# heli-sudoo/HKD-MPC

Measured on AMD Instinct MI355X. Metric: batched DDP iters/sec (fwd+bwd), 4-phase 200-knot HKD fp64, batch=4096, higher is better.
Workload: dtype f64

## Files before the change

hkd-mpc_amd/csrc/hsddp_api.cpp:

```cpp
#include <hip/hip_runtime.h>

#include <algorithm>
#include <chrono>
#include <cctype>
#include <cmath>
#include <cstdio>
#include <cstdlib>
#include <cstring>
#include <fstream>
#include <map>
#include <sstream>
#include <string>
#include <vector>

#include "../../include/hsddp.h"
#include "hsddp_internal.h"
#include "hsddp_mpc.h"

using namespace hsddp;

static thread_local std::string g_err;

static int fail(int code, const std::string &msg)
{
// ... 122 lines not shown
    if (s == "true" || s == "1") v = 1;
    else if (s == "false" || s == "0") v = 0;
    else return fail(HSDDP_ERR_IO, "conversion of data failed (" + k + ")");
    return HSDDP_OK;
}

extern "C" int hsddp_load_settings(const char *path, hsddp_options *o)
{
    if (!path || !o) return fail(HSDDP_ERR_ARG, "null argument");
    std::map<std::string, std::string> m;
    int rc = parse_info(path, m);
    if (rc) return rc;
    hsddp_options t = *o;
#define N_(k) if ((rc = get_num(m, "ddp." #k, t.k))) return rc
#define I_(k) if ((rc = get_int(m, "ddp." #k, t.k))) return rc
#define B_(k) if ((rc = get_bool(m, "ddp." #k, t.k))) return rc
    N_(alpha); N_(gamma); N_(update_penalty); N_(update_relax); N_(update_ReB);
    I_(max_DDP_iter); I_(max_AL_iter); I_(max_DDP_iter_runtime); I_(max_AL_iter_runtime);
    N_(cost_thresh); N_(tconstr_thresh); N_(pconstr_thresh); N_(dynamics_feas_thresh);
    N_(merit_rho); N_(merit_scale); N_(merit_offset);
    B_(AL_active); B_(ReB_active); B_(MS); I_(nsteps_per_node);
#undef N_
#undef I_
#undef B_
    *o = t;
    return HSDDP_OK;
}

extern "C" int hsddp_load_constraint_params(const char *path, hsddp_constraint_params *cp)
{
    if (!path || !cp) return fail(HSDDP_ERR_ARG, "null argument");
    std::map<std::string, std::string> m;
    int rc = parse_info(path, m);
    if (rc) return rc;
    hsddp_constraint_params t = *cp;
    if ((rc = get_num(m, "GRF_ReB.delta", t.grf_delta)) || (rc = get_num(m, "GRF_ReB.delta_min", t.grf_delta_min)) ||
        (rc = get_num(m, "GRF_ReB.eps", t.grf_eps)) || (rc = get_num(m, "Swing_ReB.delta", t.swing_delta)) ||
        (rc = get_num(m, "Swing_ReB.delta_min", t.swing_delta_min)) || (rc = get_num(m, "Swing_ReB.eps", t.swing_eps)) ||
        (rc = get_num(m, "TD_AL.sigma", t.td_sigma)) || (rc = get_num(m, "TD_AL.lambda", t.td_lambda)) ||
        (rc = get_num(m, "TD_AL.sigma_max", t.td_sigma_max)))
        return rc;
    *cp = t;
    return HSDDP_OK;
}

struct hsddp_handle_t {
    bool slots_fresh = false;
    bool reb_at_init = true;
    hsddp_problem_desc desc;
    hsddp_options opt;
    Params p;
    Bufs d;
    hipStream_t stream = nullptr;
    int *host_counter = nullptr;
    std::vector<hipEvent_t> events;
    struct IterGraph {
        hipGraphExec_t exec = nullptr;
        Params p;
        Bufs d;
        double alpha = 0;
        int par = 0;
    } iter_graph[8];
    int iter_graph_next = 0;
    std::vector<std::vector<int>> shift_keep;
    bool shift_overflow_pending = false;
    size_t scratch_reserved = 0;
    hipEvent_t iter_done[2] = {nullptr, nullptr};
    std::vector<void *> allocs;
    size_t bytes = 0;
    int Bref = 1;
    bool have_problem = false;
    std::vector<int> contacts;
    bool contacts_current = false;
    void *scratch = nullptr;
    size_t scratch_bytes = 0;
    std::vector<int> reach_end;
    size_t S_cap = 0;
    void *spare_K = nullptr;
    double *spare_reb_delta = nullptr, *spare_reb_eps = nullptr, *spare_al_sigma = nullptr, *spare_al_lambda = nullptr;
    int *spare_td_mask = nullptr;
    double *spare_cf_u = nullptr;
    int *spare_cf_flag = nullptr;
    double *shift_stage = nullptr;
    bool need_inputs = false;
    double *ref_table = nullptr;
    int ref_n = 0;
    float ref_dt = 0;
    bool refs_on_device = false;
    bool ref_cols_stale = true;
    std::vector<hsddp_quad_state> table_host;
    std::vector<int> win_start;
    int win_len = 0;
    float dt_sim = 0, t_cur = 0;
    std::vector<double> durations;
    int retry_cap_alloc = 0, retry_m_alloc = 0;
    float *hist = nullptr;
    std::vector<Layout> lays;
    std::vector<int> reach_el;
    double *value0 = nullptr;
    hsddp_mpc_command *cmd_dev[2] = {nullptr, nullptr}, *cmd_host[2] = {nullptr, nullptr};
    hipStream_t copy_stream = nullptr;
    hipEvent_t cmd_ready[2] = {nullptr, nullptr}, cmd_copied[2] = {nullptr, nullptr};
    char *cmd_in_host[2] = {nullptr, nullptr};
    size_t cmd_in_bytes[2] = {0, 0};
    int cmd_next = 0;
};

static int scratch(hsddp_handle h, size_t bytes, char **out)
{
    if (bytes > h->scratch_bytes) {
        if (h->scratch) hipFree(h->scratch);
        h->scratch = nullptr;
        h->scratch_bytes = 0;
        hipError_t e = hipMalloc(&h->scratch, bytes);
// ... 137 lines not shown
        p.N[i] = desc->horizons[i]; p.s0[i] = s; p.k0[i] = k;
        s += p.N[i] + 1; k += p.N[i];
    }
    p.S = s; p.Kc = k;
    p.ref_per_element = desc->ref_per_element ? 1 : 0;
    p.fp32 = desc->riccati_fp32 ? 1 : 0;
    h->Bref = p.ref_per_element ? p.B : 1;
    fill_params(h);
    for (int i = 0; i < p.P; ++i) p.ss[i] = p.N[i] + 1;
    p.has_tail = 0;
    h->reach_end.assign(p.P, 0);
    h->S_cap = (size_t)p.Kc + HSDDP_MAX_PHASES;
    const size_t B = p.B, S = h->S_cap, Kc = p.Kc, P = HSDDP_MAX_PHASES, Br = h->Bref;
    Bufs &d = h->d;
    int *contacts; double *x0, *rx, *ru, *rf;
    int rc = 0;
    if ((rc = dalloc(h, contacts, B * (P + 1) * 4)) || (rc = dalloc(h, x0, B * NX)) || (rc = dalloc(h, rx, Br * S * NX)) ||
        (rc = dalloc(h, ru, Br * S * NX)) || (rc = dalloc(h, rf, Br * S * 12)) || (rc = dalloc(h, d.ref_t, REF_COLS * Br * S)) ||
        (rc = dalloc(h, d.X3, 3 * B * S * NX)) ||
        (rc = dalloc(h, d.D3, 3 * B * S * NX)) || (rc = dalloc(h, d.U3, 3 * B * Kc * NX)) || (rc = dalloc(h, d.sel, B)) ||
        (rc = dalloc(h, d.cf_u, B * Kc * 12)) || (rc = dalloc(h, d.cf_flag, B * Kc)) ||
        (rc = dalloc(h, d.dX, B * S * NX)) ||
        (rc = dalloc(h, d.dU, B * Kc * NX)) ||
        (rc = dalloc(h, d.du, B * Kc * NX)) || (rc = dalloc(h, d.dbg, B * 16)) ||
        (p.fp32 ? ((rc = dalloc(h, d.K32, B * Kc * KCW)) || (rc = dalloc(h, d.lq32, B * Kc * LQW32)) ||
                   (rc = dalloc(h, d.def32, B * S * NX)))
                : ((rc = dalloc(h, d.K, B * Kc * KCW)) || (rc = dalloc(h, d.lq, B * Kc * LQW)))) ||
        (rc = dalloc(h, d.term, B * P * TW)) || (rc = dalloc(h, d.reb_delta, B * Kc * 20)) ||
        (rc = dalloc(h, d.reb_eps, B * Kc * 20)) || (rc = dalloc(h, d.al_sigma, B * P * MTD * 4)) ||
        (rc = dalloc(h, d.al_lambda, B * P * MTD * 4)) || (rc = dalloc(h, d.td_mask, B * P * MTD)) ||
        (rc = dalloc(h, d.term_h, B * P * 4)) ||
        (rc = dalloc(h, d.slot_cost, B * S)) || (rc = dalloc(h, d.slot_feas, B * S)) || (rc = dalloc(h, d.slot_viol, B * S)) ||
        (rc = dalloc(h, d.slot_div, B * S)) || (rc = dalloc(h, d.el, B)) || (rc = dalloc(h, d.counter, 8)) || (rc = dalloc(h, d.ls_live, LS_LIVE)) ||
        (rc = dalloc(h, (Layout *&)d.lay, B)) || (rc = dalloc(h, (int *&)d.pairs, 2 * B + 2))) {
        hsddp_destroy(h);
        return rc;
    }
    d.contacts = contacts; d.x0 = x0; d.ref_x = rx; d.ref_u = ru; d.ref_foot = rf;
    d.ref_tw = Br * S;
    d.xs3 = B * S * NX;
    d.us3 = B * Kc * NX;
    d.rows3 = (int)(B * S);
    d.urows3 = (int)(B * Kc);
    {
        const char *seq = std::getenv("HSDDP_SEQUENTIAL_RETRY");
        const char *capenv = std::getenv("HSDDP_RETRY_CAP");
        const size_t per_elem = (size_t)std::max(1, p.retry_m) * Kc * (KCW * (p.fp32 ? 4 : 8) + NX * 8 + 4);
        size_t cap = std::min<size_t>(std::min<size_t>(128, B), std::max<size_t>(2, ((size_t)256 << 20) / per_elem));
        if (capenv && std::atoi(capenv) > 0) cap = std::min<size_t>(cap, (size_t)std::atoi(capenv));
        const size_t M = (seq && seq[0] == '1') ? 0 : p.retry_m, n = cap * M;
        if (M > 0) {
            void *rk;
            if ((rc = dalloc(h, d.retry_list, cap)) || (rc = dalloc(h, d.retry_count, 1)) ||
                (rc = dalloc(h, d.retry_flag, n)) || (rc = dalloc(h, d.retry_dU, n * Kc * NX)) ||
                (rc = dalloc(h, d.retry_dv, n)) ||
                (rc = p.fp32 ? dalloc(h, (float *&)rk, n * Kc * KCW) : dalloc(h, (double *&)rk, n * Kc * KCW))) {
                hsddp_destroy(h);
                return rc;
            }
            d.retry_K = rk;
            h->retry_cap_alloc = (int)cap;
            h->retry_m_alloc = (int)M;
            fill_params(h);
        }
    }
    if (hipStreamCreateWithFlags(&h->stream, hipStreamNonBlocking) != hipSuccess ||
        hipHostMalloc((void **)&h->host_counter, 16 * sizeof(int), 0) != hipSuccess) {
        hsddp_destroy(h);
        return fail(HSDDP_ERR_DEVICE, "stream / pinned allocation failed");
    }
    if ((rc = ensure_history(h))) {
        hsddp_destroy(h);
        return rc;
    }
    launch_init_params(p, d, h->stream);
    launch_reset_elements(p, d, h->stream);
    if (hipStreamSynchronize(h->stream) != hipSuccess) {
        hsddp_destroy(h);
        return fail(HSDDP_ERR_DEVICE, "kernel launch failed at create (is the library built for this GPU?)");
    }
    *out = h;
    return HSDDP_OK;
}

extern "C" int hsddp_destroy(hsddp_handle h)
{
    if (!h) return HSDDP_OK;
    hipSetDevice(h->desc.device);
    if (h->stream) hipStreamSynchronize(h->stream);
    for (void *p : h->allocs) hipFree(p);
    if (h->scratch) hipFree(h->scratch);
    if (h->ref_table) hipFree(h->ref_table);
    if (h->hist) hipFree(h->hist);
    if (h->value0) hipFree(h->value0);

    for (auto &g : h->iter_graph)
        if (g.exec) hipGraphExecDestroy(g.exec);
    for (hipEvent_t e : h->iter_done)
        if (e) hipEventDestroy(e);
    if (h->host_counter) hipHostFree(h->host_counter);
    if (h->copy_stream) hipStreamSynchronize(h->copy_stream);
    for (int q = 0; q < 2; ++q) {
        if (h->cmd_dev[q]) hipFree(h->cmd_dev[q]);
        if (h->cmd_host[q]) hipHostFree(h->cmd_host[q]);
        if (h->cmd_ready[q]) hipEventDestroy(h->cmd_ready[q]);
        if (h->cmd_copied[q]) hipEventDestroy(h->cmd_copied[q]);
        if (h->cmd_in_host[q]) hipHostFree(h->cmd_in_host[q]);
    }
    if (h->copy_stream) hipStreamDestroy(h->copy_stream);
    for (hipEvent_t e : h->events) hipEventDestroy(e);
    if (h->stream) hipStreamDestroy(h->stream);
    delete h;
    return HSDDP_OK;
}

extern "C" int hsddp_validate_options(const hsddp_options *o)
{
    if (!o) return fail(HSDDP_ERR_ARG, "null argument");
    if (!(o->alpha > 0 && o->alpha < 1)) return fail(HSDDP_ERR_ARG, "alpha must lie in (0, 1)");
    if (o->max_AL_iter < 0 || o->max_DDP_iter < 0) return fail(HSDDP_ERR_ARG, "negative iteration budget");
    if (!(o->update_regularization > 1))
        return fail(HSDDP_ERR_ARG, "update_regularization must exceed 1 (the regularisation schedule would never end)");
    int m = 0;
    for (double mu = 0;; ++m) {
        mu = std::fmax(mu * o->update_regularization, 1e-03);
        if (mu > 1e2) break;
        if (m >= HSDDP_MAX_REG_ATTEMPTS)
            return fail(HSDDP_ERR_ARG, "update_regularization too close to 1: more than HSDDP_MAX_REG_ATTEMPTS "
                                       "regularisation retries per failed sweep");
    }
    return HSDDP_OK;
}

extern "C" int hsddp_set_options(hsddp_handle h, const hsddp_options *o)
{
    if (!h || !o) return fail(HSDDP_ERR_ARG, "null argument");
    int rc = hsddp_validate_options(o);
    if (rc) return rc;
    if (1 + (long)std::max(0, o->max_AL_iter) * std::max(0, o->max_DDP_iter) > (1L << 20))
        return fail(HSDDP_ERR_ARG, "max_AL_iter * max_DDP_iter exceeds the solver-info history (2^20 entries)");
    const hsddp_options old = h->opt;
    h->opt = *o;
    if ((rc = ensure_history(h))) {
        h->opt = old;
        return rc;
    }
    fill_params(h);
    return HSDDP_OK;
}

static int set_layouts(hsddp_handle h, const std::vector<Layout> &lays)
{
    h->slots_fresh = false;
    Params &p = h->p;
    const int B = p.B;
    int Pmax = 0, Smax = 0, tail = 0;
    for (auto &L : lays) { Pmax = std::max(Pmax, L.P); Smax = std::max(Smax, L.S); tail |= L.has_tail; }
    std::map<std::vector<int>, std::vector<int>> groups;
    for (int b = 0; b < B; ++b) {
        std::vector<int> key(lays[b].N, lays[b].N + lays[b].P);
        key.push_back(-1);
        key.insert(key.end(), lays[b].ss, lays[b].ss + lays[b].P);
        groups[key].push_back(b);
// ... 365 lines not shown
static int count_active(hsddp_handle h, int which, int &n)
{
    HIPCHK(hipMemsetAsync(h->d.counter, 0, 4 * sizeof(int), h->stream));
    launch_count(h->p, h->d, which, h->stream);
    HIPCHK(hipMemcpyAsync(h->host_counter, h->d.counter, 4 * sizeof(int), hipMemcpyDeviceToHost, h->stream));
    HIPCHK(hipStreamSynchronize(h->stream));
    n = h->host_counter[which];
    return HSDDP_OK;
}

static int solve_check(hsddp_handle h)
{
    if (!h) return fail(HSDDP_ERR_ARG, "null handle");
    if (!h->have_problem) return fail(HSDDP_ERR_ARG, "upload the problem first");
    if (h->need_inputs) return fail(HSDDP_ERR_ARG, "the layout changed (hsddp_shift): call hsddp_update_problem first");
    HIPCHK(hipSetDevice(h->desc.device));
    return HSDDP_OK;
}

static std::vector<double> ls_steps(double alpha)
{
    std::vector<double> trials;
    for (double eps = 1; eps > 1e-3; eps *= alpha) trials.push_back(eps);
    return trials;
}

static void sync_ref_columns(hsddp_handle h)
{
    if (!h->ref_cols_stale) return;
    launch_ref_columns(h->p, h->d, h->Bref, h->stream);
    h->ref_cols_stale = false;
}

static void begin_launches(hsddp_handle h)
{
    if (h->p.trace) hipMemsetAsync(h->d.dbg, 0, (size_t)h->p.B * 16 * sizeof(unsigned long long), h->stream);
    sync_ref_columns(h);
    launch_reset_elements(h->p, h->d, h->stream);
    launch_rollout(h->p, h->d, 0.0, 0, 1, -1, h->stream);
    launch_decide(h->p, h->d, 0.0, 0, 1, -1, h->stream);
    h->slots_fresh = true;
}

static void iteration_launches(hsddp_handle h, const std::vector<double> &trials, Timer &tm)
{
    const Params &p = h->p;
    const Bufs &d = h->d;
    hipStream_t st = h->stream;
    hipEvent_t e0;
    tm.begin(0, e0);
    {
        Params pl = p;
        pl.lq_slots = h->slots_fresh ? 0 : 1;
        launch_lq(pl, d, st);
    }
    tm.end(0, e0);
    tm.begin(1, e0);
    launch_riccati(p, d, st);
    tm.end(1, e0);
    if (!p.ms0) {
        tm.begin(4, e0);
        launch_lin_rollout(p, d, st);
        tm.end(4, e0);
    }
    tm.begin(2, e0);
    for (size_t t = 0; t < trials.size(); ++t) {
        launch_rollout(p, d, trials[t], t + 1 == trials.size(), 0, (int)t, st);
        launch_decide(p, d, trials[t], t + 1 == trials.size(), 0, (int)t, st);
    }
    tm.end(2, e0);
    h->slots_fresh = true;
}

static bool graphs_enabled()
{
    const char *e = std::getenv("HSDDP_NO_GRAPH");
    return !(e && *e && *e != '0');
}

static int graph_launch(hsddp_handle h, const std::vector<double> &trials, int par)
{
    Params pl = h->p;
    pl.lq_slots = h->slots_fresh ? 0 : 1;
    hsddp_handle_t::IterGraph *hit = nullptr;
    for (auto &c : h->iter_graph)
        if (c.exec && c.par == par && !std::memcmp(&c.p, &pl, sizeof(Params)) &&
            !std::memcmp(&c.d, &h->d, sizeof(Bufs)) && c.alpha == h->opt.alpha)
            hit = &c;
    if (!hit) {
        auto &g = h->iter_graph[h->iter_graph_next];
        h->iter_graph_next = (h->iter_graph_next + 1) % 8;
        if (g.exec) {
            HIPCHK(hipStreamSynchronize(h->stream));
            HIPCHK(hipGraphExecDestroy(g.exec));
        }
        g.exec = nullptr;
        HIPCHK(hipStreamBeginCapture(h->stream, hipStreamCaptureModeThreadLocal));
        Timer off{h->stream, false, &h->events};
        iteration_launches(h, trials, off);
        launch_count(h->p, h->d, 1, h->stream);
        hipError_t e = hipMemcpyAsync(h->host_counter + 8 + 4 * par, h->d.counter, 4 * sizeof(int), hipMemcpyDeviceToHost,
                               h->stream);
        hipGraph_t graph = nullptr;
        const hipError_t ec = hipStreamEndCapture(h->stream, &graph);
        if (e == hipSuccess) e = ec;
        if (e == hipSuccess) e = hipGraphInstantiate(&g.exec, graph, nullptr, nullptr, 0);
        if (graph) hipGraphDestroy(graph);
        if (e != hipSuccess) {
            g.exec = nullptr;
            return fail(HSDDP_ERR_DEVICE, std::string("iteration graph: ") + hipGetErrorString(e));
        }
        std::memcpy(&g.p, &pl, sizeof(Params));
        std::memcpy(&g.d, &h->d, sizeof(Bufs));
        g.alpha = h->opt.alpha;
        g.par = par;
        hit = &g;
    }
    if (!h->iter_done[par]) HIPCHK(hipEventCreateWithFlags(&h->iter_done[par], hipEventDisableTiming));
    HIPCHK(hipGraphLaunch(hit->exec, h->stream));
    HIPCHK(hipEventRecord(h->iter_done[par], h->stream));
    h->slots_fresh = true;
    return HSDDP_OK;
}

static int graph_wait(hsddp_handle h, int par, int &n_active)
{
    HIPCHK(hipEventSynchronize(h->iter_done[par]));
    n_active = h->host_counter[8 + 4 * par + 1];
    return HSDDP_OK;
}

static void outer_end_launches(hsddp_handle h, Timer &tm)
{
    hipEvent_t e0;
    tm.begin(3, e0);
    if (h->opt.ReB_active && !h->p.reb_uniform) {
        h->slots_fresh = false;
        h->reb_at_init = false;
    }
    if (h->opt.ReB_active) launch_reb_update(h->p, h->d, h->stream);
    launch_outer_end(h->p, h->d, h->stream);
    tm.end(3, e0);
}

static int finish_stats(hsddp_handle h, Timer &tm, hipEvent_t e0, hsddp_stats *stats, int iters, int outers, int nbwd)
{
    HIPCHK(hipGetLastError());
    HIPCHK(hipStreamSynchronize(h->stream));
    if (!stats) return HSDDP_OK;
    hipEvent_t e1;
    hipEventCreate(&e1);
    hipEventRecord(e1, h->stream);
    hipEventSynchronize(e1);
    float ms = 0;
    hipEventElapsedTime(&ms, e0, e1);
    hipEventDestroy(e0);
    hipEventDestroy(e1);
    stats->ms_total = ms;
    stats->ms_lq = tm.total(0);
    stats->ms_backward = tm.total(1);
    stats->ms_forward = tm.total(2);
    stats->ms_other = tm.total(3);
    stats->ms_linear = tm.total(4);
    stats->inner_iterations = iters;
    stats->outer_iterations = outers;
    stats->n_backward_launches = nbwd;
    HIPCHK(hipMemsetAsync(h->d.counter + 4, 0, 2 * sizeof(int), h->stream));
    launch_stat_sums(h->p, h->d, h->stream);
    HIPCHK(hipMemcpyAsync(h->host_counter + 4, h->d.counter + 4, 2 * sizeof(int), hipMemcpyDeviceToHost, h->stream));
    HIPCHK(hipStreamSynchronize(h->stream));
    stats->ls_trials = h->host_counter[4];
    stats->element_iterations = h->host_counter[5];
    return HSDDP_OK;
}

static hipEvent_t start_stats(hsddp_handle h, hsddp_stats *stats)
{
    if (!stats) return nullptr;
    memset(stats, 0, sizeof(*stats));
    hipEvent_t e0;
    hipEventCreate(&e0);
    hipEventRecord(e0, h->stream);
    return e0;
}

extern "C" int hsddp_solve(hsddp_handle h, hsddp_stats *stats)
{
    int rc = solve_check(h);
    if (rc) return rc;
    Timer tm{h->stream, stats != nullptr, &h->events};
    hipEvent_t e0 = start_stats(h, stats);
    const std::vector<double> trials = ls_steps(h->opt.alpha);
    begin_launches(h);
    int iters = 0, outers = 0, nbwd = 0;
    const bool checks = !h->opt.no_early_exit;
    const bool graph = checks && graphs_enabled();
    for (int ou = 0; ou < h->opt.max_AL_iter; ++ou) {
        tm.cut();
        launch_outer_begin(h->p, h->d, h->stream);
        outers++;
        for (int in = 0; in < h->opt.max_DDP_iter; ++in) {
            if (graph) {
                int n = 0;
                tm.cut();
                if (in == 0 && (rc = graph_launch(h, trials, 0))) return rc;
                if (in + 1 < h->opt.max_DDP_iter && (rc = graph_launch(h, trials, (in + 1) & 1))) return rc;
                if ((rc = graph_wait(h, in & 1, n))) return rc;
                iters++;
                nbwd++;
                if (n == 0) break;
                continue;
            }
            iteration_launches(h, trials, tm);
            iters++;
            nbwd++;
            if (checks) {
                int n = 0;
                tm.cut();
                if ((rc = count_active(h, 1, n))) return rc;
                if (n == 0) break;
            }
        }
        outer_end_launches(h, tm);
        if (checks) {
            int n = 0;
            tm.cut();
            if ((rc = count_active(h, 2, n))) return rc;
            if (n == 0) break;
        }
    }
    return finish_stats(h, tm, e0, stats, iters, outers, nbwd);
}

extern "C" int hsddp_solve_begin(hsddp_handle h)
{
    int rc = solve_check(h);
    if (rc) return rc;
    begin_launches(h);
    launch_outer_begin(h->p, h->d, h->stream);
    HIPCHK(hipGetLastError());
    return HSDDP_OK;
}

extern "C" int hsddp_iterate(hsddp_handle h, int n, hsddp_stats *stats)
{
    int rc = solve_check(h);
    if (rc) return rc;
    if (n < 0) return fail(HSDDP_ERR_ARG, "negative iteration count");
    Timer tm{h->stream, stats != nullptr, &h->events};
    hipEvent_t e0 = start_stats(h, stats);
    const std::vector<double> trials = ls_steps(h->opt.alpha);
    sync_ref_columns(h);
    for (int i = 0; i < n; ++i) iteration_launches(h, trials, tm);
    return finish_stats(h, tm, e0, stats, n, 0, n);
}

extern "C" int hsddp_solve_end(hsddp_handle h)
{
    int rc = solve_check(h);
    if (rc) return rc;
    Timer tm{h->stream, false, &h->events};
    outer_end_launches(h, tm);
    HIPCHK(hipGetLastError());
    HIPCHK(hipStreamSynchronize(h->stream));
    return HSDDP_OK;
}

static int d2h(void *dst, const void *src, size_t bytes)
{
    if (!dst) return HSDDP_OK;
    HIPCHK(hipMemcpy(dst, src, bytes, hipMemcpyDeviceToHost));
    return HSDDP_OK;
}

extern "C" int hsddp_download_trajectory(hsddp_handle h, double *Xbar, double *Ubar, double *K)
{
    if (!h) return fail(HSDDP_ERR_ARG, "null handle");
    HIPCHK(hipSetDevice(h->desc.device));
    HIPCHK(hipStreamSynchronize(h->stream));
    const size_t B = h->p.B, S = h->p.S, Kc = h->p.Kc;
    int rc;
    launch_normalize(h->p, h->d, h->stream);
    HIPCHK(hipStreamSynchronize(h->stream));
    if ((rc = d2h(Xbar, h->d.X3, B * S * NX * 8)) || (rc = d2h(Ubar, h->d.U3, B * Kc * NX * 8)))
        return rc;
    if (K && h->need_inputs)
        return fail(HSDDP_ERR_ARG, "the layout changed (hsddp_shift): call hsddp_update_problem before downloading K");
    if (K) {
        std::vector<double> kc(B * Kc * KCW);
        if (h->p.fp32) {
            std::vector<float> k32(B * Kc * KCW);
            if ((rc = d2h(k32.data(), h->d.K32, B * Kc * KCW * 4))) return rc;
            std::copy(k32.begin(), k32.end(), kc.begin());
        } else if ((rc = d2h(kc.data(), h->d.K, B * Kc * KCW * 8))) {
            return rc;
        }
        std::memset(K, 0, B * Kc * NN * sizeof(double));
        for (size_t b = 0; b < B; ++b)
            for (size_t k = 0; k < Kc; ++k)
                for (int q = 0; q < 12; ++q) {
                    const int u = coupled_control(h, b, k, q);
                    std::memcpy(K + ((b * Kc + k) * NX + u) * NX, &kc[((b * Kc + k) * 12 + q) * NX], NX * sizeof(double));
                }
    }
    return HSDDP_OK;
// ... 1141 lines not shown
```

hkd-mpc_amd/csrc/hsddp_internal.h:

```cpp
#pragma once

#include <hip/hip_runtime.h>
#include "hkd_model.h"

namespace hsddp {

constexpr int NX = 24;
constexpr int NN = 576;
constexpr int MAXP = 16;
constexpr int LS_LIVE = 128;
constexpr int MTD = 4;
constexpr int TD_PENDING = 0x10;
constexpr int KCW = 12 * 24;

constexpr int LQ_SE = 0;
constexpr int LQ_SW = 16;
constexpr int LQ_BW = 68;
constexpr int LQ_LX = 104;
constexpr int LQ_LU = 128;
constexpr int LQ_RB = 152;
constexpr int LQW = 176;
constexpr int LQW32 = 192;
constexpr int sw_at(int r, int q) { return LQ_SW + 3 * q + r; }
constexpr int bw_at(int r, int k) { return LQ_BW + 3 * k + r; }
// ... 26 lines not shown
    double grf_inv_delta, grf_log_delta;
    int lq_slots;
    int fp32;
    int ss[MAXP];
    int has_tail;
    int retry_cap, retry_m;
    int hcap;
    int elem_layout;
    int n_pairs;
    int store_value;
    int ms0;
    int trace;
};

struct RetryEntry {
    int b, pad;
    double reg;
};

constexpr int TD_STALE = 0x20;

struct ElemState {
    double cost, feas, merit, merit_rho, dV1, dV2, reg;
    double max_t, max_p, max_t_prev, max_p_prev, cost_prev, merit_prev, feas_prev;
    int done, inner_done, ls_active, accepted, status, iters, outer_iters, n_ls;
    int hist_n;
    int ovr, td_stale;
};

struct Bufs {
    const int *contacts;
    const double *x0;
    const double *ref_x, *ref_u, *ref_foot;
    double *ref_t;
    size_t ref_tw;
    double *X3, *D3, *dX;
    double *U3, *dU, *du;
    size_t xs3, us3;
    int rows3, urows3;
    int *sel;
    double *cf_u;
    int *cf_flag;
    double *K, *lq, *term;
    double *reb_delta, *reb_eps, *al_sigma, *al_lambda, *term_h;
    int *td_mask;
    double *slot_cost, *slot_feas, *slot_viol;
    int *slot_div;
    float *lq32, *K32, *def32;
    ElemState *el;
    int *counter;
    int *ls_live;
    RetryEntry *retry_list;
    int *retry_count, *retry_flag;
    void *retry_K;
    double *retry_dU;
    double *retry_dv;
    unsigned long long *dbg;
    float *hist;
    const Layout *lay;
    const int *pairs;
    double *value0;
};

void launch_rollout(const Params &p, const Bufs &d, double eps, int last, int init, int tix, hipStream_t st);
void launch_decide(const Params &p, const Bufs &d, double eps, int last, int init, int tix, hipStream_t st);
void launch_normalize(const Params &p, const Bufs &d, hipStream_t st);
void launch_reset_working(const Params &p, const Bufs &d, hipStream_t st);
void launch_lq(const Params &p, const Bufs &d, hipStream_t st);
void launch_riccati(const Params &p, const Bufs &d, hipStream_t st);
void launch_lin_rollout(const Params &p, const Bufs &d, hipStream_t st);
void launch_outer_begin(const Params &p, const Bufs &d, hipStream_t st);
void launch_reb_update(const Params &p, const Bufs &d, hipStream_t st);
void launch_outer_end(const Params &p, const Bufs &d, hipStream_t st);
void launch_reset_elements(const Params &p, const Bufs &d, hipStream_t st);
void launch_init_params(const Params &p, const Bufs &d, hipStream_t st);
void launch_resolve_td(const Params &p, const Bufs &d, hipStream_t st);
constexpr int REF_COLS = 24 + 24 + 12;
void launch_ref_columns(const Params &p, const Bufs &d, int Bref, hipStream_t st);
void launch_count(const Params &p, const Bufs &d, int which, hipStream_t st);
void launch_stat_sums(const Params &p, const Bufs &d, hipStream_t st);
void launch_broadcast(double *dst, const double *src, size_t n, size_t copies, hipStream_t st);

void launch_model_dynamics(const double *x, const double *u, const double *c, double dt, double *xn, int n,
                           hipStream_t st);
void launch_model_partial(const double *x, const double *u, const double *c, double dt, double *A, double *B,
                          int n, hipStream_t st);
void launch_model_foot(const double *x, const int *leg, double *p, double *J, int n, hipStream_t st);
void launch_model_reset(const double *x, const int *c, const int *cn, double *xn, double *Px, int n,
                        hipStream_t st);
void launch_model_running_cost(const Params &p, const double *x, const double *u, const int *c, const double *xr,
                               const double *ur, const double *pf, int terms, double *l, double *lx, double *lu,
                               double *lxx, double *luu, int n, hipStream_t st);
void launch_model_terminal_cost(const Params &p, const double *x, const int *c, const double *xr, const double *pf,
                                int terms, double *Phi, double *Phix, double *Phixx, int n, hipStream_t st);
void launch_model_grf(const double *u, const int *c, double mu, double *g, double *gu, int n, hipStream_t st);
void launch_model_touchdown(const double *x, const int *c, const int *cn, double ground, double *h, double *hx, int n,
                            hipStream_t st);

}
```

hkd-mpc_amd/csrc/hsddp_kernels.hip:

```cpp
#include <cstdlib>

#include "hsddp_device.h"

namespace hsddp {

using namespace hkd;

#ifndef HSDDP_STAMPS
#define HSDDP_STAMPS 0
#endif
#if HSDDP_STAMPS
#define RSTAMP(n)                                                                             \
    do {                                                                                      \
        __builtin_amdgcn_sched_barrier(0);                                                    \
        unsigned long long t_;                                                                \
        asm volatile("s_waitcnt lgkmcnt(0)\n\ts_memtime %0\n\ts_waitcnt lgkmcnt(0)" : "=s"(t_)::"memory"); \
        __builtin_amdgcn_sched_barrier(0);                                                    \
        rst[n] = t_;                                                                          \
    } while (0)
#else
#define RSTAMP(n) \
    do {          \
    } while (0)
#endif
// ... 1476 lines not shown

static bool fused_decide(const Params &p)
{
    if (p.B > 16 || p.has_tail || p.ms0) return false;
    const char *e = std::getenv("HSDDP_NO_FUSED_DECIDE");
    return !(e && *e && *e != '0');
}

void launch_rollout(const Params &p, const Bufs &d, double eps, int last, int init, int tix, hipStream_t st)
{
    if (p.ms0) {
        LAUNCH_EL(k_rollout_ss, dim3((p.B + 3) / 4), dim3(64), st, p, d, eps, init, tix);
        return;
    }
    const dim3 g(blocks_for((long)p.B * p.S, 64) + blocks_for((long)p.B * p.P, 64));
    const bool wide = p.S >= RW;
    if (fused_decide(p)) {
        if (p.elem_layout) {
            if (wide) hipLaunchKernelGGL((k_rollout<true, true, true>), g, dim3(64), 0, st, p, d, eps, init, tix, last);
            else hipLaunchKernelGGL((k_rollout<true, true, false>), g, dim3(64), 0, st, p, d, eps, init, tix, last);
        } else {
            if (wide) hipLaunchKernelGGL((k_rollout<false, true, true>), g, dim3(64), 0, st, p, d, eps, init, tix, last);
            else hipLaunchKernelGGL((k_rollout<false, true, false>), g, dim3(64), 0, st, p, d, eps, init, tix, last);
        }
        return;
    }
    if (p.elem_layout) {
        if (wide) hipLaunchKernelGGL((k_rollout<true, false, true>), g, dim3(64), 0, st, p, d, eps, init, tix, last);
        else hipLaunchKernelGGL((k_rollout<true, false, false>), g, dim3(64), 0, st, p, d, eps, init, tix, last);
    } else {
        if (wide) hipLaunchKernelGGL((k_rollout<false, false, true>), g, dim3(64), 0, st, p, d, eps, init, tix, last);
        else hipLaunchKernelGGL((k_rollout<false, false, false>), g, dim3(64), 0, st, p, d, eps, init, tix, last);
    }
    if (p.has_tail) LAUNCH_EL(k_rollout_tail, dim3((p.B + 63) / 64), dim3(64), st, p, d, eps, init, tix);
}
void launch_decide(const Params &p, const Bufs &d, double eps, int last, int init, int tix, hipStream_t st)
{
    if (fused_decide(p)) return;
    LAUNCH_EL(k_decide, dim3((p.B + 3) / 4), dim3(64), st, p, d, eps, last, init, tix);
}
void launch_normalize(const Params &p, const Bufs &d, hipStream_t st)
{
    hipLaunchKernelGGL(k_normalize, dim3(blocks_for((long)p.B * p.S * (NX / 2), 256)), dim3(256), 0, st, p, d);
    hipLaunchKernelGGL(k_normalize_sel, dim3(blocks_for(p.B, 256)), dim3(256), 0, st, p, d);
}
template <bool EL>
__global__ __launch_bounds__(128, 4) void k_terminal(Params p, Bufs d)
{
    __shared__ TermLds S[2 * TERM_TPW];
    const int w = threadIdx.x >> 6;
    terminal_wave<EL>(p, d, S + w * TERM_TPW, (long)blockIdx.x * 2 + w, threadIdx.x & 63);
}

void launch_lq(const Params &p, const Bufs &d, hipStream_t st)
{
    const unsigned nterm = blocks_for((long)p.B * p.P, 4 * TERM_TPW);
    const bool merged = nterm <= 256;
    const bool by_knot = !p.lq_slots && !p.fp32;
    if (!merged) {
        const unsigned nt2 = blocks_for((long)p.B * p.P, 2 * TERM_TPW);
        if (p.elem_layout) hipLaunchKernelGGL((k_terminal<true>), dim3(nt2), dim3(128), 0, st, p, d);
        else hipLaunchKernelGGL((k_terminal<false>), dim3(nt2), dim3(128), 0, st, p, d);
    }
    const dim3 g(blocks_for((long)p.B * (by_knot ? p.Kc : p.S), 256) + (merged ? nterm : 0));
    if (p.fp32) {
#define HSDDP_LQ(f, e)                                                          \
    do {                                                                        \
        if (p.lq_slots) hipLaunchKernelGGL((k_lq<f, e, true>), g, dim3(256), 0, st, p, d); \
        else hipLaunchKernelGGL((k_lq<f, e, false>), g, dim3(256), 0, st, p, d);           \
    } while (0)
        if (p.elem_layout) HSDDP_LQ(true, true);
        else HSDDP_LQ(true, false);
    } else {
        if (p.elem_layout) HSDDP_LQ(false, true);
        else HSDDP_LQ(false, false);
#undef HSDDP_LQ
    }
}

__global__ __launch_bounds__(256) void k_broadcast(double *dst, const double *src, size_t n, size_t total)
{
    const size_t gid = (size_t)blockIdx.x * blockDim.x + threadIdx.x;
    if (gid < total) dst[gid] = src[gid % n];
}
void launch_broadcast(double *dst, const double *src, size_t n, size_t copies, hipStream_t st)
{
    const size_t total = n * copies;
    if (total) hipLaunchKernelGGL(k_broadcast, dim3((unsigned)((total + 255) / 256)), dim3(256), 0, st, dst, src, n, total);
}

void launch_reset_working(const Params &p, const Bufs &d, hipStream_t st)
{
    hipLaunchKernelGGL(k_reset_defect, dim3(blocks_for((long)p.B * p.S * (NX / 2), 256)), dim3(256), 0, st, p, d);
    hipLaunchKernelGGL(k_reset_sel, dim3(blocks_for(p.B, 256)), dim3(256), 0, st, p, d);
}
void launch_outer_begin(const Params &p, const Bufs &d, hipStream_t st)
{
    hipLaunchKernelGGL(k_outer_begin, dim3(blocks_for(p.B, 256)), dim3(256), 0, st, p, d);
}
void launch_reb_update(const Params &p, const Bufs &d, hipStream_t st)
{
    LAUNCH_EL(k_reb_update, dim3(blocks_for((long)p.B * p.Kc, 256)), dim3(256), st, p, d);
}
void launch_outer_end(const Params &p, const Bufs &d, hipStream_t st)
{
    LAUNCH_EL(k_outer_end, dim3(blocks_for(p.B, 256)), dim3(256), st, p, d);
}
void launch_reset_elements(const Params &p, const Bufs &d, hipStream_t st)
{
    hipLaunchKernelGGL(k_reset_elements, dim3(blocks_for(p.B, 256)), dim3(256), 0, st, p, d);
}
void launch_init_params(const Params &p, const Bufs &d, hipStream_t st)
{
    long n = (long)p.B * p.Kc * 20;
    if ((long)p.B * p.P * MTD * 4 > n) n = (long)p.B * p.P * MTD * 4;
    hipLaunchKernelGGL(k_init_params, dim3(blocks_for(n, 256)), dim3(256), 0, st, p, d);
    hipLaunchKernelGGL(k_term_identity, dim3(blocks_for((long)p.B * MAXP * 12 * NX, 256)), dim3(256), 0, st, p, d);
}
void launch_resolve_td(const Params &p, const Bufs &d, hipStream_t st)
{
    LAUNCH_EL(k_resolve_td, dim3(blocks_for((long)p.B * p.P * MTD, 256)), dim3(256), st, p, d);
}
void launch_stat_sums(const Params &p, const Bufs &d, hipStream_t st)
{
    hipLaunchKernelGGL(k_stat_sums, dim3((p.B + 255) / 256), dim3(256), 0, st, p, d);
}

void launch_count(const Params &p, const Bufs &d, int which, hipStream_t st)
{
    hipLaunchKernelGGL(k_count, dim3(blocks_for(p.B, 256)), dim3(256), 0, st, p, d, which);
// ... 45 lines not shown
```

hkd-mpc_amd/csrc/hsddp_sweep.hip:

```cpp
#include "hsddp_wave.h"

namespace hsddp {

using namespace hkd;

namespace sweep {

#ifndef HSDDP_STAMPS
#define HSDDP_STAMPS 0
#endif
#ifndef SWEEP_WPB2_WPE
#define SWEEP_WPB2_WPE 1
#endif
#if HSDDP_STAMPS
#define STAMP(n)                                                                              \
    do {                                                                                      \
        __builtin_amdgcn_sched_barrier(0);                                                    \
        unsigned long long t_;                                                                \
        asm volatile("s_waitcnt lgkmcnt(0)\n\ts_memtime %0\n\ts_waitcnt lgkmcnt(0)" : "=s"(t_)::"memory"); \
        __builtin_amdgcn_sched_barrier(0);                                                    \
        if (threadIdx.x == 0) {                                                               \
            if ((n) > 0) S.st[n] += t_ - S.tprev;                                             \
            S.tprev = t_;                                                                     \
        }                                                                                     \
// ... 843 lines not shown
    double dvk = 0.0;
    for (int attempt = 0; __builtin_amdgcn_ballot_w64(need); ++attempt) {
        it.act = need;
        it.reg = (real)reg;
        double dv;
        const int fk = sweep_pair<real, EL, DV, W>(p, d, S, L, it, dv);
        if (attempt == 0 && p.retry_cap > 0) {
            if (W == 0 && need && fk >= 0 && L.pp == 0) {
                const int f = atomicAdd(d.retry_count, 1);
                if (f < p.retry_cap) d.retry_list[f] = RetryEntry{bv, 0, reg};
                S.fl[L.e] = f;
            }
            CSYNC();
        }
        if (need) {
            if (fk < 0) {
                ok = true;
                need = false;
                dvk = dv;
            } else {
                const bool deferred = attempt == 0 && p.retry_cap > 0 && S.fl[L.e] < p.retry_cap;
                if (deferred) {
                    need = false;
                    if (W == 0 && L.pp == 0) { E.iters += 1; E.cost = ecost; E.feas = efeas; E.accepted = 0; }
                    act = false;
                } else {
                    reg = fmax(reg * p.update_regularization, 1e-03);
                    if (reg > 1e2 || attempt >= MAX_REG_ATTEMPTS) need = false;
                }
            }
        }
        CSYNC();
    }
    if (W == 0 && act && L.pp == 0) {
        double rn = reg / 20;
        if (rn < 1e-06) rn = 0;
        E.iters += 1; E.cost = ecost; E.feas = efeas; E.accepted = 0;
        E.reg = rn;
        if (!ok) { E.status = 1; E.done = 1; E.ls_active = 0; }
        if (DV && ok) merit_step(p, E, dvk, -dvk);
    }
}

template <bool EL, bool DV>
__global__ __launch_bounds__(128) __attribute__((amdgpu_waves_per_eu(2))) void k_riccati_cs(Params p, Bufs d)
{
    __shared__ LdsCS<double> S;
    zero_init(S, threadIdx.x & 63);
    __syncthreads();
    if (threadIdx.x < 64) riccati_cs_wave<EL, DV, 0>(p, d, S);
    else riccati_cs_wave<EL, DV, 1>(p, d, S);
}

template <typename real, bool EL, bool DV>
__global__ __launch_bounds__(64, 2) void k_riccati_retry(Params p, Bufs d)
{
    __shared__ Lds<real> S;
    const Lane L = make_lane();
    zero_init(S, L.lane);
    const int n = min(*d.retry_count, p.retry_cap);
    const int mpad = p.retry_m + (p.retry_m & 1);
    const int item = 2 * blockIdx.x + L.e, f = item / mpad, a = item % mpad + 1;
    bool act = f < n && a <= p.retry_m;
    if (!__builtin_amdgcn_ballot_w64(act)) return;
    const int fv = f < n ? f : 0;
    const RetryEntry e = d.retry_list[fv];
    double reg = e.reg;
    for (int t = 0; t < a; ++t) reg = fmax(reg * p.update_regularization, 1e-03);
    const int av = a <= p.retry_m ? a : p.retry_m;
    int *flag = d.retry_flag + fv * p.retry_m + (av - 1);
    if (act && reg > 1e2) {
        if (L.pp == 0) *flag = 2;
        act = false;
    }
    if (!__builtin_amdgcn_ballot_w64(act)) return;
    const size_t slot = (size_t)fv * p.retry_m + (av - 1);
    Item<real> it;
    it.b = e.b;
    it.act = act;
    it.reg = (real)reg;
    it.K = (real *)d.retry_K + slot * p.Kc * KCW;
    it.dU = d.retry_dU + slot * p.Kc * NX;
    double dv;
    const int fk = sweep_pair<real, EL, DV>(p, d, S, L, it, dv);
    if (act && L.pp == 0) *flag = fk < 0 ? 1 : -1 - fk;
    if (DV && act && L.pp == 0) d.retry_dv[slot] = dv;
}

template <typename real>
__global__ __launch_bounds__(64) void k_riccati_select(Params p, Bufs d)
{
    const int f = blockIdx.x, lane = threadIdx.x;
    if (f >= min(*d.retry_count, p.retry_cap)) return;
    const RetryEntry e = d.retry_list[f];
    const size_t b = e.b;
    double reg = e.reg;
    int win = 0;
    for (int a = 1; a <= p.retry_m; ++a) {
        reg = fmax(reg * p.update_regularization, 1e-03);
        if (reg > 1e2) break;
        if (d.retry_flag[f * p.retry_m + a - 1] == 1) { win = a; break; }
    }
    real *Ko = Prec<real>::K(d) + b * p.Kc * KCW;
    double *dUo = d.dU + b * p.Kc * NX;
    if (win) {
        const size_t slot = (size_t)f * p.retry_m + (win - 1);
        const real *Ks = (const real *)d.retry_K + slot * p.Kc * KCW;
        const double *Us = d.retry_dU + slot * p.Kc * NX;
        for (size_t q = lane; q < (size_t)p.Kc * KCW; q += 64) Ko[q] = Ks[q];
        for (size_t q = lane; q < (size_t)p.Kc * NX; q += 64) dUo[q] = Us[q];
    } else {
        const int *fl = d.retry_flag + f * p.retry_m;
        auto source = [&](int kc) {
            int src = 0;
            for (int a = 1; a <= p.retry_m && fl[a - 1] != 2; ++a)
                if (-1 - fl[a - 1] < kc) src = a;
            return src;
        };
        const real *K0 = (const real *)d.retry_K + (size_t)f * p.retry_m * p.Kc * KCW;
        const double *U0 = d.retry_dU + (size_t)f * p.retry_m * p.Kc * NX;
        for (size_t q = lane; q < (size_t)p.Kc * KCW; q += 64) {
            const int a = source((int)(q / KCW));
            if (a) Ko[q] = K0[(size_t)(a - 1) * p.Kc * KCW + q];
        }
        for (size_t q = lane; q < (size_t)p.Kc * NX; q += 64) {
            const int a = source((int)(q / NX));
            if (a) dUo[q] = U0[(size_t)(a - 1) * p.Kc * NX + q];
        }
    }
    if (lane == 0) {
        ElemState &E = d.el[b];
        double rn = reg / 20;
        if (rn < 1e-06) rn = 0;
        E.reg = rn;
        if (!win) { E.status = 1; E.done = 1; E.ls_active = 0; }
        else if (p.ms0) {
            const double dv = d.retry_dv[(size_t)f * p.retry_m + (win - 1)];
            merit_step(p, E, dv, -dv);
        }
    }
}

static int device_cus()
{
    static int cus[64] = {0};
    int dev = 0;
// ... 12 lines not shown
    if (p.fp32) return false;
    const char *e = std::getenv("HSDDP_SWEEP_SPLIT");
    if (e && *e) return *e != '0';
    return (p.elem_layout ? p.n_pairs : (p.B + 1) / 2) <= device_cus();
}

static int sweep_wpb(const Params &p)
{
    if (p.fp32) return 1;
    const char *e = std::getenv("HSDDP_SWEEP_WPB");
    if (e && *e) return *e == '2' ? 2 : 1;
    const int pairs = p.elem_layout ? p.n_pairs : (p.B + 1) / 2, cus = device_cus();
    return pairs > cus && pairs <= 4 * cus ? 2 : 1;
}

void launch_riccati(const Params &p, const Bufs &d, hipStream_t st)
{
    const dim3 g1((unsigned)(p.elem_layout ? p.n_pairs : (p.B + 1) / 2));
#define HSDDP_RIC(kern, grid, real)                                                                          \
    do {                                                                                                     \
        if (p.ms0) {                                                                                         \
            if (p.elem_layout) hipLaunchKernelGGL((kern<real, true, true>), grid, dim3(64), 0, st, p, d);      \
            else hipLaunchKernelGGL((kern<real, false, true>), grid, dim3(64), 0, st, p, d);                   \
        } else {                                                                                             \
            if (p.elem_layout) hipLaunchKernelGGL((kern<real, true, false>), grid, dim3(64), 0, st, p, d);     \
            else hipLaunchKernelGGL((kern<real, false, false>), grid, dim3(64), 0, st, p, d);                  \
        }                                                                                                    \
    } while (0)
    const int wpb = sweep_wpb(p);
    const dim3 gw((unsigned)(((p.elem_layout ? p.n_pairs : (p.B + 1) / 2) + wpb - 1) / wpb));
#define HSDDP_RIC_W(real, W)                                                                                   \
    do {                                                                                                       \
        if (p.ms0) {                                                                                           \
            if (p.elem_layout) hipLaunchKernelGGL((k_riccati<real, true, true, W>), gw, dim3(64 * W), 0, st, p, d);  \
            else hipLaunchKernelGGL((k_riccati<real, false, true, W>), gw, dim3(64 * W), 0, st, p, d);               \
        } else {                                                                                               \
            if (p.elem_layout) hipLaunchKernelGGL((k_riccati<real, true, false, W>), gw, dim3(64 * W), 0, st, p, d); \
            else hipLaunchKernelGGL((k_riccati<real, false, false, W>), gw, dim3(64 * W), 0, st, p, d);              \
        }                                                                                                      \
    } while (0)
    if (p.fp32) HSDDP_RIC_W(float, 1);
    else if (sweep_split(p)) {
        if (p.ms0) {
            if (p.elem_layout) hipLaunchKernelGGL((k_riccati_cs<true, true>), g1, dim3(128), 0, st, p, d);
            else hipLaunchKernelGGL((k_riccati_cs<false, true>), g1, dim3(128), 0, st, p, d);
        } else {
            if (p.elem_layout) hipLaunchKernelGGL((k_riccati_cs<true, false>), g1, dim3(128), 0, st, p, d);
            else hipLaunchKernelGGL((k_riccati_cs<false, false>), g1, dim3(128), 0, st, p, d);
        }
    } else if (wpb == 2) HSDDP_RIC_W(double, 2);
    else HSDDP_RIC_W(double, 1);
#undef HSDDP_RIC_W
    if (p.retry_cap > 0) {
        const dim3 gr((unsigned)(p.retry_cap * (p.retry_m + (p.retry_m & 1)) / 2)), gs((unsigned)p.retry_cap);
        if (p.fp32) {
            HSDDP_RIC(k_riccati_retry, gr, float);
            hipLaunchKernelGGL(k_riccati_select<float>, gs, dim3(64), 0, st, p, d);
        } else {
            HSDDP_RIC(k_riccati_retry, gr, double);
            hipLaunchKernelGGL(k_riccati_select<double>, gs, dim3(64), 0, st, p, d);
        }
    }
#undef HSDDP_RIC
}

}
```

Baseline: 1.091 million.

## Fuse retry select into retry kernel via ticket counter; optional side-stream terminal LQ

```diff
diff --git a/hkd-mpc_amd/csrc/hsddp_api.cpp b/hkd-mpc_amd/csrc/hsddp_api.cpp
--- a/hkd-mpc_amd/csrc/hsddp_api.cpp
+++ b/hkd-mpc_amd/csrc/hsddp_api.cpp
@@ -198,6 +198,8 @@
     Params p;
     Bufs d;
     hipStream_t stream = nullptr;
+    LqSide lq_side = {nullptr, nullptr, nullptr};
+    bool lq_overlap = false;
     int *host_counter = nullptr;
     std::vector<hipEvent_t> events;
     struct IterGraph {
@@ -206,6 +208,7 @@
         Bufs d;
         double alpha = 0;
         int par = 0;
+        bool lq_overlap = false;
     } iter_graph[8];
     int iter_graph_next = 0;
     std::vector<std::vector<int>> shift_keep;
@@ -449,7 +452,8 @@
         if (M > 0) {
             void *rk;
             if ((rc = dalloc(h, d.retry_list, cap)) || (rc = dalloc(h, d.retry_count, 1)) ||
-                (rc = dalloc(h, d.retry_flag, n)) || (rc = dalloc(h, d.retry_dU, n * Kc * NX)) ||
+                (rc = dalloc(h, d.retry_flag, n)) || (rc = dalloc(h, d.retry_ticket, cap)) ||
+                (rc = dalloc(h, d.retry_dU, n * Kc * NX)) ||
                 (rc = dalloc(h, d.retry_dv, n)) ||
                 (rc = p.fp32 ? dalloc(h, (float *&)rk, n * Kc * KCW) : dalloc(h, (double *&)rk, n * Kc * KCW))) {
                 hsddp_destroy(h);
@@ -462,6 +466,9 @@
         }
     }
     if (hipStreamCreateWithFlags(&h->stream, hipStreamNonBlocking) != hipSuccess ||
+        hipStreamCreateWithFlags(&h->lq_side.side, hipStreamNonBlocking) != hipSuccess ||
+        hipEventCreateWithFlags(&h->lq_side.fork, hipEventDisableTiming) != hipSuccess ||
+        hipEventCreateWithFlags(&h->lq_side.join, hipEventDisableTiming) != hipSuccess ||
         hipHostMalloc((void **)&h->host_counter, 16 * sizeof(int), 0) != hipSuccess) {
         hsddp_destroy(h);
         return fail(HSDDP_ERR_DEVICE, "stream / pinned allocation failed");
@@ -506,6 +513,9 @@
     }
     if (h->copy_stream) hipStreamDestroy(h->copy_stream);
     for (hipEvent_t e : h->events) hipEventDestroy(e);
+    if (h->lq_side.fork) hipEventDestroy(h->lq_side.fork);
+    if (h->lq_side.join) hipEventDestroy(h->lq_side.join);
+    if (h->lq_side.side) hipStreamDestroy(h->lq_side.side);
     if (h->stream) hipStreamDestroy(h->stream);
     delete h;
     return HSDDP_OK;
@@ -977,7 +987,7 @@
     {
         Params pl = p;
         pl.lq_slots = h->slots_fresh ? 0 : 1;
-        launch_lq(pl, d, st);
+        launch_lq(pl, d, st, h->lq_overlap ? &h->lq_side : nullptr);
     }
     tm.end(0, e0);
     tm.begin(1, e0);
@@ -1003,6 +1013,12 @@
     return !(e && *e && *e != '0');
 }
 
+static bool lq_overlap_enabled()
+{
+    const char *e = std::getenv("HSDDP_LQ_OVERLAP");
+    return e && *e && *e != '0';
+}
+
 static int graph_launch(hsddp_handle h, const std::vector<double> &trials, int par)
 {
     Params pl = h->p;
@@ -1010,7 +1026,7 @@
     hsddp_handle_t::IterGraph *hit = nullptr;
     for (auto &c : h->iter_graph)
         if (c.exec && c.par == par && !std::memcmp(&c.p, &pl, sizeof(Params)) &&
-            !std::memcmp(&c.d, &h->d, sizeof(Bufs)) && c.alpha == h->opt.alpha)
+            !std::memcmp(&c.d, &h->d, sizeof(Bufs)) && c.alpha == h->opt.alpha && c.lq_overlap == h->lq_overlap)
             hit = &c;
     if (!hit) {
         auto &g = h->iter_graph[h->iter_graph_next];
@@ -1039,6 +1055,7 @@
         std::memcpy(&g.d, &h->d, sizeof(Bufs));
         g.alpha = h->opt.alpha;
         g.par = par;
+        g.lq_overlap = h->lq_overlap;
         hit = &g;
     }
     if (!h->iter_done[par]) HIPCHK(hipEventCreateWithFlags(&h->iter_done[par], hipEventDisableTiming));
@@ -1120,6 +1137,7 @@
     int iters = 0, outers = 0, nbwd = 0;
     const bool checks = !h->opt.no_early_exit;
     const bool graph = checks && graphs_enabled();
+    h->lq_overlap = lq_overlap_enabled();
     for (int ou = 0; ou < h->opt.max_AL_iter; ++ou) {
         tm.cut();
         launch_outer_begin(h->p, h->d, h->stream);
@@ -1176,6 +1194,7 @@
     hipEvent_t e0 = start_stats(h, stats);
     const std::vector<double> trials = ls_steps(h->opt.alpha);
     sync_ref_columns(h);
+    h->lq_overlap = lq_overlap_enabled();
     for (int i = 0; i < n; ++i) iteration_launches(h, trials, tm);
     return finish_stats(h, tm, e0, stats, n, 0, n);
 }
diff --git a/hkd-mpc_amd/csrc/hsddp_internal.h b/hkd-mpc_amd/csrc/hsddp_internal.h
--- a/hkd-mpc_amd/csrc/hsddp_internal.h
+++ b/hkd-mpc_amd/csrc/hsddp_internal.h
@@ -102,6 +102,7 @@
     int *ls_live;
     RetryEntry *retry_list;
     int *retry_count, *retry_flag;
+    int *retry_ticket;
     void *retry_K;
     double *retry_dU;
     double *retry_dv;
@@ -116,7 +117,11 @@
 void launch_decide(const Params &p, const Bufs &d, double eps, int last, int init, int tix, hipStream_t st);
 void launch_normalize(const Params &p, const Bufs &d, hipStream_t st);
 void launch_reset_working(const Params &p, const Bufs &d, hipStream_t st);
-void launch_lq(const Params &p, const Bufs &d, hipStream_t st);
+struct LqSide {
+    hipStream_t side;
+    hipEvent_t fork, join;
+};
+void launch_lq(const Params &p, const Bufs &d, hipStream_t st, const LqSide *ov = nullptr);
 void launch_riccati(const Params &p, const Bufs &d, hipStream_t st);
 void launch_lin_rollout(const Params &p, const Bufs &d, hipStream_t st);
 void launch_outer_begin(const Params &p, const Bufs &d, hipStream_t st);
diff --git a/hkd-mpc_amd/csrc/hsddp_kernels.hip b/hkd-mpc_amd/csrc/hsddp_kernels.hip
--- a/hkd-mpc_amd/csrc/hsddp_kernels.hip
+++ b/hkd-mpc_amd/csrc/hsddp_kernels.hip
@@ -1552,15 +1552,22 @@
     terminal_wave<EL>(p, d, S + w * TERM_TPW, (long)blockIdx.x * 2 + w, threadIdx.x & 63);
 }
 
-void launch_lq(const Params &p, const Bufs &d, hipStream_t st)
+void launch_lq(const Params &p, const Bufs &d, hipStream_t st, const LqSide *ov)
 {
     const unsigned nterm = blocks_for((long)p.B * p.P, 4 * TERM_TPW);
     const bool merged = nterm <= 256;
     const bool by_knot = !p.lq_slots && !p.fp32;
+    const bool fork = !merged && ov;
     if (!merged) {
         const unsigned nt2 = blocks_for((long)p.B * p.P, 2 * TERM_TPW);
-        if (p.elem_layout) hipLaunchKernelGGL((k_terminal<true>), dim3(nt2), dim3(128), 0, st, p, d);
-        else hipLaunchKernelGGL((k_terminal<false>), dim3(nt2), dim3(128), 0, st, p, d);
+        hipStream_t ts = st;
+        if (fork) {
+            hipEventRecord(ov->fork, st);
+            hipStreamWaitEvent(ov->side, ov->fork, 0);
+            ts = ov->side;
+        }
+        if (p.elem_layout) hipLaunchKernelGGL((k_terminal<true>), dim3(nt2), dim3(128), 0, ts, p, d);
+        else hipLaunchKernelGGL((k_terminal<false>), dim3(nt2), dim3(128), 0, ts, p, d);
     }
     const dim3 g(blocks_for((long)p.B * (by_knot ? p.Kc : p.S), 256) + (merged ? nterm : 0));
     if (p.fp32) {
@@ -1576,6 +1583,10 @@
         else HSDDP_LQ(false, false);
 #undef HSDDP_LQ
     }
+    if (fork) {
+        hipEventRecord(ov->join, ov->side);
+        hipStreamWaitEvent(st, ov->join, 0);
+    }
 }
 
 __global__ __launch_bounds__(256) void k_broadcast(double *dst, const double *src, size_t n, size_t total)
diff --git a/hkd-mpc_amd/csrc/hsddp_sweep.hip b/hkd-mpc_amd/csrc/hsddp_sweep.hip
--- a/hkd-mpc_amd/csrc/hsddp_sweep.hip
+++ b/hkd-mpc_amd/csrc/hsddp_sweep.hip
@@ -919,17 +919,32 @@
     else riccati_cs_wave<EL, DV, 1>(p, d, S);
 }
 
+template <typename real>
+DEV void riccati_select(const Params &p, const Bufs &d, int f, int lane);
+
+template <typename real>
+DEV void retry_finish(const Params &p, const Bufs &d, int f, int mpad, int lane)
+{
+    __threadfence();
+    int t = 0;
+    if (lane == 0) t = atomicAdd(&d.retry_ticket[f], 1);
+    if (__builtin_amdgcn_readfirstlane(t) != mpad / 2 - 1) return;
+    __threadfence();
+    riccati_select<real>(p, d, f, lane);
+    if (lane == 0) d.retry_ticket[f] = 0;
+}
+
 template <typename real, bool EL, bool DV>
 __global__ __launch_bounds__(64, 2) void k_riccati_retry(Params p, Bufs d)
 {
     __shared__ Lds<real> S;
     const Lane L = make_lane();
-    zero_init(S, L.lane);
     const int n = min(*d.retry_count, p.retry_cap);
     const int mpad = p.retry_m + (p.retry_m & 1);
     const int item = 2 * blockIdx.x + L.e, f = item / mpad, a = item % mpad + 1;
     bool act = f < n && a <= p.retry_m;
     if (!__builtin_amdgcn_ballot_w64(act)) return;
+    zero_init(S, L.lane);
     const int fv = f < n ? f : 0;
     const RetryEntry e = d.retry_list[fv];
     double reg = e.reg;
@@ -940,7 +955,10 @@
         if (L.pp == 0) *flag = 2;
         act = false;
     }
-    if (!__builtin_amdgcn_ballot_w64(act)) return;
+    if (!__builtin_amdgcn_ballot_w64(act)) {
+        retry_finish<real>(p, d, f, mpad, L.lane);
+        return;
+    }
     const size_t slot = (size_t)fv * p.retry_m + (av - 1);
     Item<real> it;
     it.b = e.b;
@@ -952,13 +970,12 @@
     const int fk = sweep_pair<real, EL, DV>(p, d, S, L, it, dv);
     if (act && L.pp == 0) *flag = fk < 0 ? 1 : -1 - fk;
     if (DV && act && L.pp == 0) d.retry_dv[slot] = dv;
+    retry_finish<real>(p, d, f, mpad, L.lane);
 }
 
 template <typename real>
-__global__ __launch_bounds__(64) void k_riccati_select(Params p, Bufs d)
-{
-    const int f = blockIdx.x, lane = threadIdx.x;
-    if (f >= min(*d.retry_count, p.retry_cap)) return;
+DEV void riccati_select(const Params &p, const Bufs &d, int f, int lane)
+{
     const RetryEntry e = d.retry_list[f];
     const size_t b = e.b;
     double reg = e.reg;
@@ -1077,14 +1094,9 @@
     else HSDDP_RIC_W(double, 1);
 #undef HSDDP_RIC_W
     if (p.retry_cap > 0) {
-        const dim3 gr((unsigned)(p.retry_cap * (p.retry_m + (p.retry_m & 1)) / 2)), gs((unsigned)p.retry_cap);
-        if (p.fp32) {
-            HSDDP_RIC(k_riccati_retry, gr, float);
-            hipLaunchKernelGGL(k_riccati_select<float>, gs, dim3(64), 0, st, p, d);
-        } else {
-            HSDDP_RIC(k_riccati_retry, gr, double);
-            hipLaunchKernelGGL(k_riccati_select<double>, gs, dim3(64), 0, st, p, d);
-        }
+        const dim3 gr((unsigned)(p.retry_cap * (p.retry_m + (p.retry_m & 1)) / 2));
+        if (p.fp32) HSDDP_RIC(k_riccati_retry, gr, float);
+        else HSDDP_RIC(k_riccati_retry, gr, double);
     }
 #undef HSDDP_RIC
 }
```

Result: no change. 1.089 million (median of 2 runs) (-0.2%).
